# NVIDIA/cuopt

Measured on NVIDIA H100. Metric: pdlp_iterations_per_sec, higher is better.
Workload: dtype f64

## Files before the change

### cuopt_b200/csrc/pdlp_kernels.cuh

```cuda
#pragma once

#include "device_utils.cuh"
#include "spmv_bicsr.cuh"

#include <math_constants.h>

namespace cuopt_b200 {

constexpr int EW_THREADS  = 256;
static __device__ int g_l2_hints = 1;

struct pdhg_ctl_t {
  double step_size, primal_weight, tau, sigma;
  double pending_weight;
  double sum_weights;
  double interaction, norm_dx2, norm_dy2;
  double reduction_exponent, growth_exponent, primal_smoothing, dual_smoothing;
  int parity;
  int pending_avg;
  int active;
  int valid;
  int k_pdhg;
  int attempts;
  int accepted;
// ... 161 lines not shown
  const bool pending      = ctl->pending_avg != 0;
  const double w          = ctl->pending_weight;
  const int stride        = gridDim.x * blockDim.x;
  const l2_policy_t pol   = make_l2_policies(g_l2_hints);
  for (int j = blockIdx.x * blockDim.x + threadIdx.x; j < n; j += stride) {
    const double xj = x[j];
    if (pending) sum_x[j] = sum_x[j] + w * xj;
    const double gradient = ld_stream(c + j) - aty[j];
    double next           = xj - (tau * gradient);
    next                  = fmax(fmin(next, ld_stream(u + j)), ld_stream(l + j));
    xn[j]                 = next;
    st_l2(xbar + j, next - xj + next, pol.keep);
  }
}

template <bool INIT, int NPRE, bool BCAST = false>
__global__ void __launch_bounds__(BICSR_THREADS, bicsr_min_ctas(NPRE)) k_dual_step(pdhg_ctl_t* __restrict__ ctl,
                                                                             bicsr_view_t A,
                                                                             const double* __restrict__ xbar,
                                                                             double* __restrict__ ybuf0,
                                                                             double* __restrict__ ybuf1,
                                                                             const double* __restrict__ lc,
                                                                             const double* __restrict__ uc,
                                                                             double* __restrict__ sum_y,
                                                                             double* __restrict__ part_dy2,
                                                                             const unsigned long long* xbar_flags,
                                                                             int n_xbar_flags,
                                                                             const double* __restrict__ t,
                                                                             peer_ptrs_t y_peers = peer_ptrs_t{},
                                                                             peer_flags_t flags = peer_flags_t{},
                                                                             int world = 1,
// ... 32 lines not shown
    const double low = next + sigma * p.lc;
    const double up  = next + sigma * p.uc;
    next             = fmax(low, fmin(up, 0.0));
    st_l2(yn + i, next, pol.keep);
    if constexpr (BCAST) {
#pragma unroll
      for (int r = 0; r < DIST_MAX_PEERS; ++r)
        if (r < world) {
          const int d = __ldg(send + (size_t)r * send_stride + i);
          if (d >= 0) y_peers.p[r][d] = next;
        }
    }
    const double d   = next - p.y;
    dy2 += d * d;
  };
  spmv_bicsr_rows<payload_t, INIT, NPRE>(A, xbar, rows[threadIdx.x >> 5], pre_op, row_op, pol.keep);
  const double tot = block_reduce(dy2, red);
  if (threadIdx.x == 0) part_dy2[blockIdx.x] = tot;
  if constexpr (BCAST) peer_signal_grid_done(&ctl->ticket[2], flags, world, DIST_FLAG_Y + rank, epoch, DIST_FLAG_Y_B + rank);
}

template <bool INIT, int NPRE>
__global__ void __launch_bounds__(BICSR_THREADS, bicsr_min_ctas(NPRE)) k_transpose_step(pdhg_ctl_t* __restrict__ ctl,
                                                                                  bicsr_view_t AT,
                                                                                  const double* __restrict__ ybuf0,
                                                                                  const double* __restrict__ ybuf1,
                                                                                  const double* __restrict__ xbuf0,
                                                                                  const double* __restrict__ xbuf1,
                                                                                  double* __restrict__ aty0,
                                                                                  double* __restrict__ aty1,
                                                                                  double* __restrict__ parts,
                                                                                  const double* __restrict__ part_dy2,
                                                                                  int n_part_dy2,
                                                                                  const double* __restrict__ t)
{
  if (!ctl->active) return;
  __shared__ double rows[BICSR_WARPS][BICSR_SLOTS];
// ... 9 lines not shown
  struct payload_t {
    double dx, aty, init;
  };
  auto pre_op = [&](int j) {
    payload_t p;
    p.dx   = ld_l2(xn + j, pol.stream) - ld_l2(x + j, pol.stream);
    p.aty  = ld_l2(aty + j, pol.stream);
    p.init = INIT ? ld_l2(t + j, pol.stream) : 0.0;
    return p;
  };
  auto row_op = [&](int j, double s, const payload_t& p) {
    st_l2(atyn + j, s, pol.stream);
    acc[0] += p.dx * (s - p.aty);
    acc[1] += p.dx * p.dx;
  };
  spmv_bicsr_rows<payload_t, INIT, NPRE>(AT, yn, rows[threadIdx.x >> 5], pre_op, row_op, pol.keep);

  if (!publish_and_elect<2>(acc, parts, &ctl->ticket[0], red)) return;
  const double interaction = gather_partials(parts, gridDim.x, red);
  const double dx2         = gather_partials(parts + gridDim.x, gridDim.x, red);
  const double dy2         = gather_partials(part_dy2, n_part_dy2, red);
  if (threadIdx.x != 0) return;

  pdhg_step_rule(ctl, interaction, dx2, dy2);
}

template <bool INIT, int NPRE>
__global__ void __launch_bounds__(BICSR_THREADS, bicsr_min_ctas(NPRE)) k_transpose_step_slice(pdhg_ctl_t* __restrict__ ctl,
                                                                                        bicsr_view_t AT,
                                                                                        const double* __restrict__ yfull,
                                                                                        const double* __restrict__ xbuf0,
// ... 334 lines not shown
__global__ void k_step_rule_gather(pdhg_ctl_t* __restrict__ ctl, const double* __restrict__ scal, int n_src,
                                   const unsigned long long* wait_flags)
{
  if (!ctl->active) return;
  if (wait_flags) peer_wait(wait_flags, n_src, (unsigned long long)ctl->attempts + 1ull);
  if (threadIdx.x != 0) return;
  double interaction = 0.0, dx2 = 0.0, dy2 = 0.0;
  for (int g = 0; g < n_src; ++g) {
    interaction += __ldcg(scal + 4 * g + 0);
    dx2 += __ldcg(scal + 4 * g + 1);
    dy2 += __ldcg(scal + 4 * g + 2);
  }
  pdhg_step_rule(ctl, interaction, dx2, dy2);
}

__global__ void __launch_bounds__(BICSR_THREADS, BICSR_MIN_CTAS) k_block_pass(const pdhg_ctl_t* __restrict__ ctl,
                                                                              bicsr_view_t Ab,
                                                                              const double* __restrict__ x0,
                                                                              const double* __restrict__ x1,
                                                                              int pick_candidate,
                                                                              double* __restrict__ t,
                                                                              int first,
                                                                              const unsigned long long* wait_flags,
                                                                              int n_wait)
{
  if (!ctl->active) return;
  __shared__ double rows[BICSR_WARPS][BICSR_SLOTS];
  if (wait_flags) peer_wait(wait_flags, n_wait, (unsigned long long)ctl->attempts + 1ull);
  const double* x       = pick_candidate ? (ctl->parity ? x0 : x1) : x0;
  const l2_policy_t pol = make_l2_policies(g_l2_hints);
  struct payload_t {
    double init;
  };
  auto pre_op = [&](int r) {
    payload_t p;
    p.init = first ? 0.0 : ld_l2(t + r, pol.stream);
    return p;
  };
  auto row_op = [&](int r, double s, const payload_t&) { st_l2(t + r, s, pol.stream); };
  spmv_bicsr_rows<payload_t, true>(Ab, x, rows[threadIdx.x >> 5], pre_op, row_op, pol.keep);
}

__global__ void __launch_bounds__(EW_THREADS) k_flush_average(const pdhg_ctl_t* __restrict__ ctl,
                                                              int n,
                                                              const double* __restrict__ xbuf0,
                                                              const double* __restrict__ xbuf1,
                                                              double* __restrict__ sum_x,
                                                              int m,
                                                              const double* __restrict__ ybuf0,
                                                              const double* __restrict__ ybuf1,
                                                              double* __restrict__ sum_y)
{
  if (!ctl->pending_avg) return;
  const int cur    = ctl->parity;
  const double* x  = cur ? xbuf1 : xbuf0;
// ... 10 lines not shown
  ctl->valid  = 0;
  ctl->active = steps > 0 ? 1 : 0;
}

__global__ void __launch_bounds__(BICSR_THREADS, BICSR_MIN_CTAS) k_spmv(bicsr_view_t A,
                                                                        const double* __restrict__ x,
                                                                        double* __restrict__ out)
{
  __shared__ double rows[BICSR_WARPS][BICSR_SLOTS];
  struct payload_t {};
  auto pre_op = [&](int) { return payload_t{}; };
  auto row_op = [&](int i, double s, const payload_t&) { out[i] = s; };
  spmv_bicsr_rows<payload_t>(A, x, rows[threadIdx.x >> 5], pre_op, row_op, make_l2_policies(g_l2_hints).keep);
}

__global__ void __launch_bounds__(BICSR_THREADS, BICSR_MIN_CTAS) k_spmv_pair(bicsr_view_t M,
                                                                             const double* __restrict__ u,
                                                                             const double* __restrict__ v,
                                                                             double* __restrict__ out_u,
                                                                             double* __restrict__ out_v,
                                                                             int first)
{
  __shared__ double rows[2][BICSR_WARPS][BICSR_SLOTS];
  auto row_op = [&](int r, double su, double sv) {
    out_u[r] = first ? su : out_u[r] + su;
    out_v[r] = first ? sv : out_v[r] + sv;
  };
  const int w = threadIdx.x >> 5;
  spmv_bicsr_rows_pair(M, u, v, rows[0][w], rows[1][w], row_op, make_l2_policies(g_l2_hints).keep);
}

__device__ __forceinline__ double bound_value_product(double value, double lower, double upper)
{
  double bound = 0.0;
  if (value > 0.0) bound = lower;
  else if (value < 0.0) bound = upper;
  return isfinite(bound) ? value * bound : 0.0;
}

__device__ __forceinline__ void eval_column(int j, const double (&s)[2], double cj, double lo, double hi,
                                            const double (&xv)[2], int reduced_cost_rule, double* __restrict__ rc_cur,
                                            double* __restrict__ rc_avg, double (&acc)[8])
{
  double* rcs[2] = {rc_cur, rc_avg};
// ... 525 lines not shown
```

### cuopt_b200/csrc/pdlp_solver.cu

```cuda
#include "pdlp_solver.hpp"

#include "dist_comm.hpp"
#include "pdlp_kernels.cuh"
#include "presolve.cuh"
#include "trust_region.cuh"

#include <math_constants.h>
#include <nvtx3/nvToolsExt.h>

#include <algorithm>
#include <chrono>
#include <cmath>
#include <cstdio>
#include <cstdlib>
#include <atomic>
#include <map>
#include <mutex>
#include <thread>
#include <string>

namespace cuopt_b200 {

namespace {

struct bicsr_dev_t {
  int n_std = 0, n_blk = 0;
  dvec<int2> desc;
  dvec<unsigned short> row_slot;
  dvec<int> idx;
  dvec<double> val;
};

struct csr_dev_t {
  int rows = 0, cols = 0, nnz = 0;
  dvec<int> off, idx;
  dvec<double> val;
  bicsr_dev_t bi;
  const csr_dev_t* structure = nullptr;
  const int* off_ptr() const { return structure ? structure->off.data() : off.data(); }
  const int* idx_ptr() const { return structure ? structure->idx.data() : idx.data(); }
  const bicsr_dev_t& bi_structure() const { return structure ? structure->bi : bi; }
  int n_blk() const { return bi_structure().n_blk; }
  bicsr_view_t view() const
  {
    const bicsr_dev_t& s = bi_structure();
    return bicsr_view_t{s.desc.data(), s.row_slot.data(), s.idx.data(), bi.val.data(), s.n_std, s.n_blk,
                        off_ptr(),     idx_ptr(),         val.data()};
  }
  void alias_structure_copy_values(const csr_dev_t& o, cudaStream_t s)
  {
    rows = o.rows; cols = o.cols; nnz = o.nnz;
    structure = &o;
    val.copy_from(o.val, s);
  }
};

constexpr int SCHEDULE_SEGMENT = 1 << 16;
template <typename T, typename F>
std::vector<T> cut_in_segments(int rows, F cut_segment)
{
  const int n_seg = std::max(1, (rows + SCHEDULE_SEGMENT - 1) / SCHEDULE_SEGMENT);
  std::vector<std::vector<T>> part(n_seg);
// ... 55 lines not shown
  if (n_std > 0) {
    const int grid = std::max(1, std::min((n_std + 7) / 8, sms * 8));
    k_bicsr_fill<<<grid, 256, 0, s>>>(n_std, b.desc.data(), d.off.data(), d.idx.data(), d.val.data(), b.idx.data(),
                                      b.val.data(), b.row_slot.data());
    CUOPT_CUDA_TRY(cudaGetLastError());
  }
}
void fill_bicsr_values(csr_dev_t& d, cudaStream_t s, int sms)
{
  const bicsr_dev_t& st = d.bi_structure();
  d.bi.val.resize((size_t)std::max(st.n_std, 1) * BICSR_SLOTS);
  if (st.n_std > 0) {
    const int grid = std::max(1, std::min((st.n_std + 7) / 8, sms * 8));
    k_bicsr_fill_values<<<grid, 256, 0, s>>>(st.n_std, st.desc.data(), d.off_ptr(), d.val.data(), d.bi.val.data());
    CUOPT_CUDA_TRY(cudaGetLastError());
  }
}

template <typename VI, typename VD>
void upload_csr(csr_dev_t& d, int rows, int cols, const VI& off, const VI& idx, const VD& val, cudaStream_t s, int sms);

}

void csr_transpose_device(int rows, int cols, int nnz, const int* off, const int* idx, const double* val, int* toff,
                          int* tidx, double* tval, cudaStream_t stream);

void sort_keys_with_index(int count, const double* keys_in, double* keys_out, const int* vals_in, int* vals_out,
                          cudaStream_t stream);
void inclusive_sum_in_place(int count, double* values, cudaStream_t stream);
void exclusive_sum_int(int count, const int* in, int* out, cudaStream_t stream);
// ... 199 lines not shown
  void* xbar_peer[DIST_MAX_PEERS]  = {};
  void* scal_peer[DIST_MAX_PEERS]  = {};
  void* flag_peer[DIST_MAX_PEERS]  = {};
  bool peers_open = false;
  peer_ptrs_t p_xbar{}, p_scal{};
  peer_flags_t p_flags{};
  dvec<unsigned> d_ticket;
  dvec<pdhg_ctl_t> d_ctl;
  dvec<eval_t> d_eval;
  pdhg_ctl_t* h_ctl = nullptr;
  eval_t* h_eval    = nullptr;
  double* h_scalar  = nullptr;
  int occ_spmv = 1;
  int occ_spmv2 = 1;
  int npre_override = 0;
  dvec<double> eval_m, eval_n;
  dvec<double> part_max;
  dvec<double> part_infeas;
  bool tr_enabled = false;
  double tr_gap_reduction_last_trial = 1.0;
  int grid_tr = 1;
  dvec<double> tr_aty, tr_ax, tr_grad, tr_dir, tr_thr, tr_thr_sorted, tr_A, tr_B, tr_parts, tr_scal;
  dvec<int> tr_iota, tr_perm;
  struct tr_gap_t {
    const double *px, *py;
    double pd = 0, dd = 0, dist = 0, lower = 0, upper = 0, ngap = 0;
  };
  struct gather_blocks_t {
    int B = 1, width = 0;
    std::vector<csr_dev_t> blk;
    std::vector<csr_dev_t> unscaled;
    std::vector<int> grid;
    bool on() const { return B > 1; }
  };
  gather_blocks_t blkA, blkAT, blkATslice;
  dvec<double> t_m, t_n;
  size_t gather_block_bytes = 0;
  int n_part_dy2 = 1;
  int grid_k1 = 1, grid_k2 = 1, grid_k3 = 1, grid_n = 1, grid_m = 1, grid_misc = 1;
  long long staged_fills = 0;
  std::map<int, cudaGraphExec_t> graphs;
  bool use_graphs = true;
  cudaEvent_t ev_a = nullptr, ev_b = nullptr;

// ... 231 lines not shown
    }
    grid_k2   = spmv_grid(As);
    grid_k3   = spmv_grid(ATs);
    grid_n    = ew_grid(n, sms);
    grid_m    = ew_grid(m, sms);
    grid_k1   = grid_n;
    grid_misc = ew_grid(std::max(n, m), sms);
    part_dy2.resize((size_t)std::max({grid_k2, grid_m, sms * 16}));
    n_part_dy2 = grid_k2;
    {
      int l2 = 0;
      CUOPT_CUDA_TRY(cudaDeviceGetAttribute(&l2, cudaDevAttrL2CacheSize, dev));
      gather_block_bytes = (size_t)((double)l2 * GATHER_BLOCK_L2_FRACTION);
    }
    if (const char* e = std::getenv("CUOPT_B200_GATHER_BLOCK_BYTES")) gather_block_bytes = (size_t)std::atoll(e);
    part_k3.resize(2 * (size_t)std::max({grid_k3, grid_n, sms * 16}));
    part_rows.resize(6 * (size_t)grid_m);
    if (hp.restart_strategy == 2) {
      tr_enabled = true;
      {
        if (sharded())
          throw lp_error(error_type_t::ValidationError, "Methodical1 is not available in multi-GPU solves");
        const size_t N = (size_t)n + m;
        grid_tr        = ew_grid((int)std::min<size_t>(N, 1u << 30), sms);
        tr_aty.resize(n); tr_ax.resize(m); tr_grad.resize(N); tr_dir.resize(N); tr_thr.resize(N); tr_thr_sorted.resize(N);
        tr_A.resize(N); tr_B.resize(N); tr_iota.resize(N); tr_perm.resize(N);
        tr_parts.resize(5 * (size_t)grid_tr);
        tr_scal.resize(TR_SCALARS);
        tr_scal.zero(stream);
      }
// ... 462 lines not shown
    g = gather_blocks_t{};
    const size_t bytes = (size_t)M.cols * sizeof(double);
    int B              = 1;
    if (forced_width > 0) {
      if (M.nnz == 0 || M.rows == 0) return;
      g.width = forced_width;
      B       = 2;
    } else {
      if (gather_block_bytes == 0 || bytes <= gather_block_bytes + gather_block_bytes / 2 || M.nnz == 0) return;
      B       = (int)std::min<size_t>(16, (bytes + gather_block_bytes - 1) / gather_block_bytes);
      g.width = (((M.cols + B - 1) / B) + 31) & ~31;
      B       = (M.cols + g.width - 1) / g.width;
    }
    if (B <= 1) return;
    g.B = B;
    g.blk.resize(B);
    std::vector<int*> offs(B), idxs(B);
    std::vector<double*> vals(B);
    std::vector<int> nnz_b(B, 0);
    for (int b = 0; b < B; ++b) {
      g.blk[b].rows = M.rows;
      g.blk[b].cols = M.cols;
      g.blk[b].off.resize((size_t)M.rows + 1);
      offs[b] = g.blk[b].off.data();
    }
    csr_split_columns_offsets(M.rows, M.off_ptr(), M.idx_ptr(), g.width, B, offs.data(), nnz_b.data(), stream);
    for (int b = 0; b < B; ++b) {
      g.blk[b].nnz = nnz_b[b];
      g.blk[b].idx.resize((size_t)nnz_b[b]);
      g.blk[b].val.resize((size_t)nnz_b[b]);
      idxs[b] = g.blk[b].idx.data();
      vals[b] = g.blk[b].val.data();
    }
    csr_split_columns_fill(M.rows, M.off_ptr(), M.idx_ptr(), M.val.data(), g.width, B, offs.data(), idxs.data(), vals.data(),
                           stream);
    std::vector<int> hoff((size_t)M.rows + 1);
    g.grid.resize(B);
    for (int b = 0; b < B; ++b) {
      g.blk[b].off.download(hoff.data(), stream);
      sync();
      build_bicsr(g.blk[b], hoff, stream, sms);
      g.grid[b] = spmv_grid(g.blk[b]);
    }
    if (unscaled_src) {
      g.unscaled.resize(B);
      for (int b = 0; b < B; ++b) {
        csr_dev_t& U = g.unscaled[b];
        U.rows = M.rows; U.cols = M.cols; U.nnz = nnz_b[b];
        U.structure = &g.blk[b];
        U.val.resize((size_t)nnz_b[b]);
        vals[b] = U.val.data();
      }
      csr_split_columns_fill(M.rows, M.off_ptr(), M.idx_ptr(), unscaled_src->val.data(), g.width, B, offs.data(), idxs.data(),
                             vals.data(), stream);
      for (csr_dev_t& U : g.unscaled) {
        fill_bicsr_values(U, stream, sms);
        if (U.bi_structure().n_std == U.bi_structure().n_blk) {
          sync();
          U.val = dvec<double>{};
        }
      }
    }
    t.resize((size_t)M.rows);
    t.zero(stream);
  }
  void launch_block_passes(const gather_blocks_t& g, int count, const double* x0, const double* x1, int pick_candidate,
                           double* t, const unsigned long long* wait_flags, int n_wait)
  {
    for (int b = 0; b < count; ++b) {
      const csr_dev_t& M = g.blk[b];
      k_block_pass<<<g.grid[b], BICSR_THREADS, 0, stream>>>(d_ctl.data(), M.view(), x0, x1, pick_candidate, t, b == 0,
                                                            b == 0 ? wait_flags : nullptr, n_wait);
    }
  }
  void enqueue_k2(const unsigned long long* wait_flags, int n_wait, bool bcast = false,
                  const unsigned long long* wait_flags_b = nullptr)
  {
    const bool blocked  = blkA.on();
    const csr_dev_t& L  = blocked ? blkA.blk[blkA.B - 1] : hot_A();
    const int npre      = fused_npre(L);
    const int grid      = spmv_grid(L, npre);
    const double* t     = blocked ? t_m.data() : nullptr;
    const unsigned long long* wf = wait_flags_b ? wait_flags_b : (blocked ? nullptr : wait_flags);
    if (blocked) launch_block_passes(blkA, blkA.B - 1, xbar.data(), xbar.data(), 0, t_m.data(), wait_flags, n_wait);
#define CUOPT_K2(INIT, NPRE)                                                                                             \
  k_dual_step<INIT, NPRE><<<grid, BICSR_THREADS, 0, stream>>>(d_ctl.data(), L.view(), xbar.data(), ybuf[0].data(),       \
                                                              ybuf[1].data(), lcs.data(), ucs.data(), sum_y.data(),      \
                                                              part_dy2.data(), wf, n_wait, t)
#define CUOPT_K2B(INIT, NPRE)                                                                                            \
  k_dual_step<INIT, NPRE, true><<<grid, BICSR_THREADS, 0, stream>>>(d_ctl.data(), L.view(), xbar.data(), ybuf[0].data(), \
                                                                    ybuf[1].data(), lcs.data(), ucs.data(), sum_y.data(), \
                                                                    part_dy2.data(), wf, n_wait, t, p_yfull, p_flags,     \
                                                                    dist->world, dist->rank, sendY.data(), m)
    if (bcast) {
      if (blocked) { if (npre > 1) CUOPT_K2B(true, 2); else CUOPT_K2B(true, 1); }
      else { if (npre > 1) CUOPT_K2B(false, 2); else CUOPT_K2B(false, 1); }
    } else if (blocked) { if (npre > 1) CUOPT_K2(true, 2); else CUOPT_K2(true, 1); }
    else { if (npre > 1) CUOPT_K2(false, 2); else CUOPT_K2(false, 1); }
#undef CUOPT_K2B
#undef CUOPT_K2
  }
  int k2_grid() const
  {
    const csr_dev_t& L = blkA.on() ? blkA.blk[blkA.B - 1] : hot_A();
    return spmv_grid(L, fused_npre(L));
  }
  int k3_npre() const { return npre_override > 1 ? 2 : 1; }
  int k3_grid() const { return spmv_grid(blkAT.on() ? blkAT.blk[blkAT.B - 1] : ATs, k3_npre()); }
  void enqueue_k3()
  {
    const bool blocked = blkAT.on();
    const csr_dev_t& L = blocked ? blkAT.blk[blkAT.B - 1] : ATs;
    const int npre     = k3_npre();
    const int grid     = k3_grid();
    const double* t    = blocked ? t_n.data() : nullptr;
    if (blocked) launch_block_passes(blkAT, blkAT.B - 1, ybuf[0].data(), ybuf[1].data(), 1, t_n.data(), nullptr, 0);
#define CUOPT_K3(INIT, NPRE)                                                                                              \
  k_transpose_step<INIT, NPRE><<<grid, BICSR_THREADS, 0, stream>>>(d_ctl.data(), L.view(), ybuf[0].data(), ybuf[1].data(), \
                                                                   xbuf[0].data(), xbuf[1].data(), atybuf[0].data(),      \
                                                                   atybuf[1].data(), part_k3.data(), part_dy2.data(),     \
                                                                   n_part_dy2, t)
    if (blocked) { if (npre > 1) CUOPT_K3(true, 2); else CUOPT_K3(true, 1); }
    else { if (npre > 1) CUOPT_K3(false, 2); else CUOPT_K3(false, 1); }
#undef CUOPT_K3
  }
  int kernels_per_attempt() const
  {
    const int k2 = blkA.on() ? blkA.B : 1;
    if (!sharded()) return 1 + k2 + (blkAT.on() ? blkAT.B : 1);
    if (dist_gather) return 1 + k2 + (blkATslice.on() ? blkATslice.B : 1) + 1 + (dist_send_kernel ? 2 : 0);
    return 1 + k2 + (blkAT.on() ? blkAT.B : 1) + 2;
  }

  void launch_transpose_partial()
  {
    if (blkAT.on()) {
      launch_block_passes(blkAT, blkAT.B, ybuf[0].data(), ybuf[1].data(), 1, dist_buf.data(), nullptr, 0);
      return;
    }
    k_transpose_partial<<<grid_k3, BICSR_THREADS, 0, stream>>>(d_ctl.data(), ATs.view(), ybuf[0].data(), ybuf[1].data(),
                                                               dist_buf.data());
  }
  void launch_spmv(const csr_dev_t& M, const double* v, double* out)
  {
    k_spmv<<<spmv_grid(M), BICSR_THREADS, 0, stream>>>(M.view(), v, out);
  }
  int launch_spmv_pair(const csr_dev_t& M, const gather_blocks_t& g, const double* u, const double* v, double* out_u,
                       double* out_v)
  {
    const int count = g.unscaled.empty() ? 1 : (int)g.unscaled.size();
    for (int b = 0; b < count; ++b) {
      const csr_dev_t& Mb = g.unscaled.empty() ? M : g.unscaled[b];
      k_spmv_pair<<<spmv_grid(Mb), BICSR_THREADS, 0, stream>>>(Mb.view(), u, v, out_u, out_v, b == 0);
    }
    return count;
  }

  void enqueue_sliced_attempt()
  {
    const int j0 = slice_j0, G = dist->world, rk = dist->rank;
    double *x0 = xbuf[0].data() + j0, *x1 = xbuf[1].data() + j0, *a0 = atybuf[0].data() + j0, *a1 = atybuf[1].data() + j0;
    if (dist_gather) {
      const unsigned long long* fl = d_flags.data();
      tr_tick(0);
      if (dist_send_kernel) {
        k_primal_step<<<grid_slice, EW_THREADS, 0, stream>>>(d_ctl.data(), slice_n, x0, x1, a0, a1, cs.data() + j0,
                                                             ls.data() + j0, us.data() + j0, sum_x.data() + j0, xloc.data());
        CUOPT_CUDA_TRY(cudaEventRecord(ev_fork, stream));
// ... 710 lines not shown
  if (name == "sum_w") return k.sum_weights;
  if (name == "k_total") return s.total_pdlp_iterations;
  if (name == "k_pdhg") return k.attempts;
  if (name == "its_since_restart") return k.its_since_restart;
  if (name == "interaction") return k.interaction;
  if (name == "norm_dx2") return k.norm_dx2;
  if (name == "norm_dy2") return k.norm_dy2;
  if (name == "l2_norm_b") return s.l2_norm_b;
  if (name == "l2_norm_c") return s.l2_norm_c;
  if (name == "last_restart_kkt") return s.last_restart_kkt;
  if (name == "last_candidate_kkt") return s.last_candidate_kkt;
  if (name == "n_restarts") return s.sol.stats.n_restarts;
  if (name == "last_restart_was_average") return s.last_restart_was_average ? 1.0 : 0.0;
  if (name == "eval_blocks") return (double)std::max<size_t>(1, s.blkA.unscaled.size());
  if (name == "eval_blocks_t") return (double)std::max<size_t>(1, s.blkAT.unscaled.size());
  if (name == "valid") return k.valid;
  if (name == "sm_count") return s.sms;
  if (name == "occ_spmv") return s.occ_spmv;
  if (name == "occ_spmv2") return s.occ_spmv2;
  if (name == "grid_k1") return s.grid_k1;
  if (name == "grid_k2") return s.k2_grid();
  if (name == "grid_k3") return s.k3_grid();
  if (name == "grid_n") return s.grid_n;
  if (name == "grid_m") return s.grid_m;
  if (name == "k2_npre") return s.fused_npre(s.blkA.on() ? s.blkA.blk[s.blkA.B - 1] : s.hot_A());
  if (name == "n_std_a") return s.As.bi_structure().n_std;
  if (name == "n_blk_a") return s.As.bi_structure().n_blk;
  if (name == "n_std_at") return s.ATs.bi_structure().n_std;
  if (name == "n_blk_at") return s.ATs.bi_structure().n_blk;
  if (name == "staged_fills") return (double)s.staged_fills;
// ... 163 lines not shown
```

### cuopt_b200/csrc/spmv_bicsr.cuh

```cuda
#pragma once

#include "device_utils.cuh"

namespace cuopt_b200 {

constexpr int BICSR_CH              = 8;
constexpr int BICSR_SLOTS           = 32 * BICSR_CH;
constexpr int BICSR_MAX_ROWS        = 256;
constexpr int BICSR_THREADS         = 256;
constexpr int BICSR_WARPS           = BICSR_THREADS / 32;
constexpr int BICSR_PAD             = 0x7fffffff;
constexpr unsigned short BICSR_EMPTY = 0xffff;
constexpr int BICSR_MIN_CTAS        = 4;
__host__ __device__ constexpr int bicsr_min_ctas(int npre) { return npre > 1 ? 3 : BICSR_MIN_CTAS; }

__host__ __device__ constexpr int bicsr_slot(int q) { return (q % BICSR_CH) * 32 + q / BICSR_CH; }

struct bicsr_view_t {
  const int2* desc;
  const unsigned short* row_slot;
  const int* idx;
  const double* val;
  int n_std, n_blk;
  const int* off;
  const int* cidx;
  const double* cval;
};

__device__ __forceinline__ void bicsr_block_row_sums(const double (&a)[BICSR_CH], const double (&g)[BICSR_CH], unsigned ends,
                                                     int lane, double* rsw)
{
  constexpr unsigned FULL = 0xffffffffu;
  double s = 0.0, head = 0.0;
  const int kf = ends ? __ffs(ends) - 1 : -1;
#pragma unroll
  for (int k = 0; k < BICSR_CH; ++k) {
    s = __dadd_rn(s, __dmul_rn(a[k], g[k]));
    const bool e = (ends >> k) & 1u;
    if (e && k != kf) rsw[k * 32 + lane] = s;
    head = (k == kf) ? s : head;
    s    = e ? 0.0 : s;
  }
  double tail  = s;
  double carry = __shfl_up_sync(FULL, tail, 1);
  if (lane == 0) carry = 0.0;
  unsigned pending = __ballot_sync(FULL, kf < 0);
  while (pending) {
    if (kf < 0) tail = carry + s;
    carry = __shfl_up_sync(FULL, tail, 1);
    if (lane == 0) carry = 0.0;
    pending &= pending << 1;
  }
  if (kf >= 0) rsw[kf * 32 + lane] = carry + head;
}

template <typename P, bool INIT = false, int NPRE = 1, typename PreOp, typename RowOp>
__device__ __forceinline__ void spmv_bicsr_rows(const bicsr_view_t& A,
                                                const double* __restrict__ x,
                                                double* rsw,
                                                PreOp& pre_op,
                                                RowOp& row_op,
                                                unsigned long long gather_policy)
{
  const int lane          = threadIdx.x & 31;
  const int gwarp         = blockIdx.x * BICSR_WARPS + (threadIdx.x >> 5);
  const int nwarps        = gridDim.x * BICSR_WARPS;
  int c[BICSR_CH];
  if (gwarp < A.n_std) {
#pragma unroll
    for (int k = 0; k < BICSR_CH; ++k) c[k] = ld_stream(A.idx + (size_t)gwarp * BICSR_SLOTS + k * 32 + lane);
  }
  for (int b = gwarp; b < A.n_std; b += nwarps) {
    const int2 d  = __ldg(A.desc + b);
    const int r0 = d.x, r1 = d.y;
    P pl[NPRE];
    unsigned short slot[NPRE];
#pragma unroll
    for (int q = 0; q < NPRE; ++q) {
      slot[q] = BICSR_EMPTY;
      if (r0 + lane + 32 * q < r1) {
        pl[q]   = pre_op(r0 + lane + 32 * q);
        slot[q] = __ldg(A.row_slot + r0 + lane + 32 * q);
      }
    }
    const size_t base = (size_t)b * BICSR_SLOTS + lane;
    double a[BICSR_CH], g[BICSR_CH];
#pragma unroll
    for (int k = 0; k < BICSR_CH; ++k) a[k] = ld_stream(A.val + base + k * 32);
#pragma unroll
    for (int k = 0; k < BICSR_CH; ++k) {
      const int col = c[k] & 0x7fffffff;
      g[k]          = col != BICSR_PAD ? ld_l2(x + col, gather_policy) : 0.0;
    }
    unsigned ends = 0;
#pragma unroll
    for (int k = 0; k < BICSR_CH; ++k) ends |= (unsigned)(c[k] < 0) << k;
    if (b + nwarps < A.n_std) {
#pragma unroll
      for (int k = 0; k < BICSR_CH; ++k) c[k] = ld_stream(A.idx + (size_t)(b + nwarps) * BICSR_SLOTS + k * 32 + lane);
    }
    bicsr_block_row_sums(a, g, ends, lane, rsw);
    __syncwarp();
#pragma unroll
    for (int q = 0; q < NPRE; ++q) {
      if (r0 + lane + 32 * q < r1) {
        double sum = slot[q] != BICSR_EMPTY ? rsw[slot[q]] : 0.0;
        if constexpr (INIT) sum = pl[q].init + sum;
        row_op(r0 + lane + 32 * q, sum, pl[q]);
      }
    }
    for (int r = r0 + 32 * NPRE + lane; r < r1; r += 32) {
      const P p2              = pre_op(r);
      const unsigned short s2 = __ldg(A.row_slot + r);
      double sum              = s2 != BICSR_EMPTY ? rsw[s2] : 0.0;
      if constexpr (INIT) sum = p2.init + sum;
      row_op(r, sum, p2);
    }
    __syncwarp();
  }
  for (int b = A.n_std + gwarp; b < A.n_blk; b += nwarps) {
    const int row = __ldg(A.desc + b).x;
    const int lo = __ldg(A.off + row), hi = __ldg(A.off + row + 1);
    P pl;
    if (lane == 0) pl = pre_op(row);
    double acc = 0.0;
    for (int e = lo + lane; e < hi; e += 32) acc += ld_stream(A.cval + e) * ld_l2(x + ld_stream(A.cidx + e), gather_policy);
    acc = warp_sum(acc);
    if (lane == 0) {
      if constexpr (INIT) acc = pl.init + acc;
      row_op(row, acc, pl);
    }
  }
}

template <typename RowOp>
__device__ __forceinline__ void spmv_bicsr_rows_pair(const bicsr_view_t& A,
                                                     const double* __restrict__ u,
                                                     const double* __restrict__ v,
                                                     double* rsw_u,
                                                     double* rsw_v,
                                                     RowOp& row_op,
                                                     unsigned long long gather_policy)
{
  const int lane   = threadIdx.x & 31;
  const int gwarp  = blockIdx.x * BICSR_WARPS + (threadIdx.x >> 5);
  const int nwarps = gridDim.x * BICSR_WARPS;
  for (int b = gwarp; b < A.n_std; b += nwarps) {
    const int2 d      = __ldg(A.desc + b);
    const size_t base = (size_t)b * BICSR_SLOTS + lane;
    int c[BICSR_CH];
    double a[BICSR_CH], gu[BICSR_CH], gv[BICSR_CH];
#pragma unroll
    for (int k = 0; k < BICSR_CH; ++k) c[k] = ld_stream(A.idx + base + k * 32);
#pragma unroll
    for (int k = 0; k < BICSR_CH; ++k) a[k] = ld_stream(A.val + base + k * 32);
#pragma unroll
    for (int k = 0; k < BICSR_CH; ++k) {
      const int col = c[k] & 0x7fffffff;
      gu[k]         = col != BICSR_PAD ? ld_l2(u + col, gather_policy) : 0.0;
      gv[k]         = col != BICSR_PAD ? ld_l2(v + col, gather_policy) : 0.0;
    }
    unsigned ends = 0;
#pragma unroll
    for (int k = 0; k < BICSR_CH; ++k) ends |= (unsigned)(c[k] < 0) << k;
    bicsr_block_row_sums(a, gu, ends, lane, rsw_u);
    bicsr_block_row_sums(a, gv, ends, lane, rsw_v);
    __syncwarp();
    for (int r = d.x + lane; r < d.y; r += 32) {
      const unsigned short s = __ldg(A.row_slot + r);
      row_op(r, s != BICSR_EMPTY ? rsw_u[s] : 0.0, s != BICSR_EMPTY ? rsw_v[s] : 0.0);
    }
    __syncwarp();
  }
  for (int b = A.n_std + gwarp; b < A.n_blk; b += nwarps) {
    const int row = __ldg(A.desc + b).x;
    const int lo = __ldg(A.off + row), hi = __ldg(A.off + row + 1);
    double acc_u = 0.0, acc_v = 0.0;
    for (int e = lo + lane; e < hi; e += 32) {
      const double a = ld_stream(A.cval + e);
      const int col  = ld_stream(A.cidx + e);
      acc_u += a * ld_l2(u + col, gather_policy);
      acc_v += a * ld_l2(v + col, gather_policy);
    }
    acc_u = warp_sum(acc_u);
    acc_v = warp_sum(acc_v);
// ... 43 lines not shown
{
  const int lane = threadIdx.x & 31, wpb = blockDim.x >> 5;
  for (int b = blockIdx.x * wpb + (threadIdx.x >> 5); b < n_std; b += gridDim.x * wpb) {
    const int2 d      = desc[b];
    const int lo      = off[d.x];
    const int cnt     = off[d.y] - lo;
    const size_t base = (size_t)b * BICSR_SLOTS;
#pragma unroll
    for (int k = 0; k < BICSR_CH; ++k) {
      const int q                = BICSR_CH * lane + k;
      bval[base + k * 32 + lane] = q < cnt ? val[lo + q] : 0.0;
    }
  }
}

}
```

Baseline: 366.1.

## Compact block-CSR column indices to 24-bit and replace row slots with bitmasks

```diff
diff --git a/cuopt_b200/csrc/pdlp_kernels.cuh b/cuopt_b200/csrc/pdlp_kernels.cuh
--- a/cuopt_b200/csrc/pdlp_kernels.cuh
+++ b/cuopt_b200/csrc/pdlp_kernels.cuh
@@ -199,7 +199,7 @@
   }
 }
 
-template <bool INIT, int NPRE, bool BCAST = false>
+template <bool INIT, int NPRE, bool BCAST = false, int FMT = 0>
 __global__ void __launch_bounds__(BICSR_THREADS, bicsr_min_ctas(NPRE)) k_dual_step(pdhg_ctl_t* __restrict__ ctl,
                                                                              bicsr_view_t A,
                                                                              const double* __restrict__ xbar,
@@ -262,13 +262,13 @@
     const double d   = next - p.y;
     dy2 += d * d;
   };
-  spmv_bicsr_rows<payload_t, INIT, NPRE>(A, xbar, rows[threadIdx.x >> 5], pre_op, row_op, pol.keep);
+  spmv_bicsr_rows<payload_t, INIT, NPRE, FMT>(A, xbar, rows[threadIdx.x >> 5], pre_op, row_op, pol.keep);
   const double tot = block_reduce(dy2, red);
   if (threadIdx.x == 0) part_dy2[blockIdx.x] = tot;
   if constexpr (BCAST) peer_signal_grid_done(&ctl->ticket[2], flags, world, DIST_FLAG_Y + rank, epoch, DIST_FLAG_Y_B + rank);
 }
 
-template <bool INIT, int NPRE>
+template <bool INIT, int NPRE, int FMT = 0>
 __global__ void __launch_bounds__(BICSR_THREADS, bicsr_min_ctas(NPRE)) k_transpose_step(pdhg_ctl_t* __restrict__ ctl,
                                                                                   bicsr_view_t AT,
                                                                                   const double* __restrict__ ybuf0,
@@ -308,7 +308,7 @@
     acc[0] += p.dx * (s - p.aty);
     acc[1] += p.dx * p.dx;
   };
-  spmv_bicsr_rows<payload_t, INIT, NPRE>(AT, yn, rows[threadIdx.x >> 5], pre_op, row_op, pol.keep);
+  spmv_bicsr_rows<payload_t, INIT, NPRE, FMT>(AT, yn, rows[threadIdx.x >> 5], pre_op, row_op, pol.keep);
 
   if (!publish_and_elect<2>(acc, parts, &ctl->ticket[0], red)) return;
   const double interaction = gather_partials(parts, gridDim.x, red);
@@ -673,6 +673,7 @@
   pdhg_step_rule(ctl, interaction, dx2, dy2);
 }
 
+template <int FMT = 0>
 __global__ void __launch_bounds__(BICSR_THREADS, BICSR_MIN_CTAS) k_block_pass(const pdhg_ctl_t* __restrict__ ctl,
                                                                               bicsr_view_t Ab,
                                                                               const double* __restrict__ x0,
@@ -697,7 +698,7 @@
     return p;
   };
   auto row_op = [&](int r, double s, const payload_t&) { st_l2(t + r, s, pol.stream); };
-  spmv_bicsr_rows<payload_t, true>(Ab, x, rows[threadIdx.x >> 5], pre_op, row_op, pol.keep);
+  spmv_bicsr_rows<payload_t, true, 1, FMT>(Ab, x, rows[threadIdx.x >> 5], pre_op, row_op, pol.keep);
 }
 
 __global__ void __launch_bounds__(EW_THREADS) k_flush_average(const pdhg_ctl_t* __restrict__ ctl,
@@ -738,6 +739,7 @@
   spmv_bicsr_rows<payload_t>(A, x, rows[threadIdx.x >> 5], pre_op, row_op, make_l2_policies(g_l2_hints).keep);
 }
 
+template <int FMT = 0>
 __global__ void __launch_bounds__(BICSR_THREADS, BICSR_MIN_CTAS) k_spmv_pair(bicsr_view_t M,
                                                                              const double* __restrict__ u,
                                                                              const double* __restrict__ v,
@@ -751,7 +753,7 @@
     out_v[r] = first ? sv : out_v[r] + sv;
   };
   const int w = threadIdx.x >> 5;
-  spmv_bicsr_rows_pair(M, u, v, rows[0][w], rows[1][w], row_op, make_l2_policies(g_l2_hints).keep);
+  spmv_bicsr_rows_pair<FMT>(M, u, v, rows[0][w], rows[1][w], row_op, make_l2_policies(g_l2_hints).keep);
 }
 
 __device__ __forceinline__ double bound_value_product(double value, double lower, double upper)
diff --git a/cuopt_b200/csrc/pdlp_solver.cu b/cuopt_b200/csrc/pdlp_solver.cu
--- a/cuopt_b200/csrc/pdlp_solver.cu
+++ b/cuopt_b200/csrc/pdlp_solver.cu
@@ -25,10 +25,14 @@
 
 struct bicsr_dev_t {
   int n_std = 0, n_blk = 0;
+  int fmt = 0, col0 = 0;
   dvec<int2> desc;
   dvec<unsigned short> row_slot;
   dvec<int> idx;
   dvec<double> val;
+  dvec<unsigned short> lo16;
+  dvec<unsigned long long> hi8;
+  dvec<unsigned> mask;
 };
 
 struct csr_dev_t {
@@ -44,8 +48,8 @@
   bicsr_view_t view() const
   {
     const bicsr_dev_t& s = bi_structure();
-    return bicsr_view_t{s.desc.data(), s.row_slot.data(), s.idx.data(), bi.val.data(), s.n_std, s.n_blk,
-                        off_ptr(),     idx_ptr(),         val.data()};
+    return bicsr_view_t{s.desc.data(), s.row_slot.data(), s.idx.data(), bi.val.data(), s.n_std,  s.n_blk, off_ptr(),
+                        idx_ptr(),     val.data(),        s.lo16.data(), s.hi8.data(), s.mask.data(), s.col0};
   }
   void alias_structure_copy_values(const csr_dev_t& o, cudaStream_t s)
   {
@@ -131,6 +135,38 @@
     const int grid = std::max(1, std::min((st.n_std + 7) / 8, sms * 8));
     k_bicsr_fill_values<<<grid, 256, 0, s>>>(st.n_std, st.desc.data(), d.off_ptr(), d.val.data(), d.bi.val.data());
     CUOPT_CUDA_TRY(cudaGetLastError());
+  }
+}
+
+void compact_bicsr(csr_dev_t& d, int fmt, int col0, cudaStream_t s, int sms)
+{
+  bicsr_dev_t& b = d.bi;
+  b.fmt  = fmt;
+  b.col0 = col0;
+  if (fmt == 0 || b.n_std == 0) return;
+  const size_t ns = (size_t)b.n_std;
+  if (fmt & BICSR_FMT_IDX3) {
+    b.lo16.resize(ns * BICSR_SLOTS);
+    b.hi8.resize(ns * 32);
+  }
+  if (fmt & BICSR_FMT_MASK) b.mask.resize(ns * 8);
+  const int grid = std::max(1, std::min((b.n_std + BICSR_WARPS - 1) / BICSR_WARPS, sms * 8));
+  k_bicsr_fill_structure<<<grid, BICSR_THREADS, 0, s>>>(b.n_std, b.desc.data(), d.off.data(), d.idx.data(), col0,
+                                                        b.lo16.data(), b.hi8.data(), b.mask.data());
+  CUOPT_CUDA_TRY(cudaGetLastError());
+  CUOPT_CUDA_TRY(cudaStreamSynchronize(s));
+  if (fmt & BICSR_FMT_IDX3) b.idx = dvec<int>{};
+  if (fmt & BICSR_FMT_MASK) b.row_slot = dvec<unsigned short>{};
+}
+
+template <typename F>
+void with_fmt(int fmt, F&& f)
+{
+  switch (fmt) {
+    case BICSR_FMT_IDX3: f(std::integral_constant<int, BICSR_FMT_IDX3>{}); break;
+    case BICSR_FMT_MASK: f(std::integral_constant<int, BICSR_FMT_MASK>{}); break;
+    case BICSR_FMT_IDX3 | BICSR_FMT_MASK: f(std::integral_constant<int, BICSR_FMT_IDX3 | BICSR_FMT_MASK>{}); break;
+    default: f(std::integral_constant<int, 0>{});
   }
 }
 
@@ -360,6 +396,7 @@
   int occ_spmv = 1;
   int occ_spmv2 = 1;
   int npre_override = 0;
+  int compact_blocks = BICSR_FMT_IDX3 | BICSR_FMT_MASK;
   dvec<double> eval_m, eval_n;
   dvec<double> part_max;
   dvec<double> part_infeas;
@@ -374,6 +411,7 @@
   };
   struct gather_blocks_t {
     int B = 1, width = 0;
+    int fmt = 0;
     std::vector<csr_dev_t> blk;
     std::vector<csr_dev_t> unscaled;
     std::vector<int> grid;
@@ -635,6 +673,7 @@
       gather_block_bytes = (size_t)((double)l2 * GATHER_BLOCK_L2_FRACTION);
     }
     if (const char* e = std::getenv("CUOPT_B200_GATHER_BLOCK_BYTES")) gather_block_bytes = (size_t)std::atoll(e);
+    if (const char* e = std::getenv("CUOPT_B200_COMPACT_BLOCKS")) compact_blocks = std::atoi(e) & (BICSR_FMT_IDX3 | BICSR_FMT_MASK);
     part_k3.resize(2 * (size_t)std::max({grid_k3, grid_n, sms * 16}));
     part_rows.resize(6 * (size_t)grid_m);
     if (hp.restart_strategy == 2) {
@@ -1127,6 +1166,10 @@
     }
     if (B <= 1) return;
     g.B = B;
+    if (forced_width == 0 && !sharded()) {
+      g.fmt = compact_blocks;
+      if (g.width > BICSR_IDX3_MAX_WIDTH) g.fmt &= ~BICSR_FMT_IDX3;
+    }
     g.blk.resize(B);
     std::vector<int*> offs(B), idxs(B);
     std::vector<double*> vals(B);
@@ -1153,6 +1196,7 @@
       g.blk[b].off.download(hoff.data(), stream);
       sync();
       build_bicsr(g.blk[b], hoff, stream, sms);
+      compact_bicsr(g.blk[b], g.fmt, b * g.width, stream, sms);
       g.grid[b] = spmv_grid(g.blk[b]);
     }
     if (unscaled_src) {
@@ -1182,8 +1226,10 @@
   {
     for (int b = 0; b < count; ++b) {
       const csr_dev_t& M = g.blk[b];
-      k_block_pass<<<g.grid[b], BICSR_THREADS, 0, stream>>>(d_ctl.data(), M.view(), x0, x1, pick_candidate, t, b == 0,
-                                                            b == 0 ? wait_flags : nullptr, n_wait);
+      with_fmt(g.fmt, [&](auto F) {
+        k_block_pass<decltype(F)::value><<<g.grid[b], BICSR_THREADS, 0, stream>>>(
+          d_ctl.data(), M.view(), x0, x1, pick_candidate, t, b == 0, b == 0 ? wait_flags : nullptr, n_wait);
+      });
     }
   }
   void enqueue_k2(const unsigned long long* wait_flags, int n_wait, bool bcast = false,
@@ -1196,10 +1242,10 @@
     const double* t     = blocked ? t_m.data() : nullptr;
     const unsigned long long* wf = wait_flags_b ? wait_flags_b : (blocked ? nullptr : wait_flags);
     if (blocked) launch_block_passes(blkA, blkA.B - 1, xbar.data(), xbar.data(), 0, t_m.data(), wait_flags, n_wait);
-#define CUOPT_K2(INIT, NPRE)                                                                                             \
-  k_dual_step<INIT, NPRE><<<grid, BICSR_THREADS, 0, stream>>>(d_ctl.data(), L.view(), xbar.data(), ybuf[0].data(),       \
-                                                              ybuf[1].data(), lcs.data(), ucs.data(), sum_y.data(),      \
-                                                              part_dy2.data(), wf, n_wait, t)
+#define CUOPT_K2(INIT, NPRE, FMT)                                                                                        \
+  k_dual_step<INIT, NPRE, false, FMT><<<grid, BICSR_THREADS, 0, stream>>>(                                               \
+    d_ctl.data(), L.view(), xbar.data(), ybuf[0].data(), ybuf[1].data(), lcs.data(), ucs.data(), sum_y.data(),          \
+    part_dy2.data(), wf, n_wait, t)
 #define CUOPT_K2B(INIT, NPRE)                                                                                            \
   k_dual_step<INIT, NPRE, true><<<grid, BICSR_THREADS, 0, stream>>>(d_ctl.data(), L.view(), xbar.data(), ybuf[0].data(), \
                                                                     ybuf[1].data(), lcs.data(), ucs.data(), sum_y.data(), \
@@ -1208,8 +1254,11 @@
     if (bcast) {
       if (blocked) { if (npre > 1) CUOPT_K2B(true, 2); else CUOPT_K2B(true, 1); }
       else { if (npre > 1) CUOPT_K2B(false, 2); else CUOPT_K2B(false, 1); }
-    } else if (blocked) { if (npre > 1) CUOPT_K2(true, 2); else CUOPT_K2(true, 1); }
-    else { if (npre > 1) CUOPT_K2(false, 2); else CUOPT_K2(false, 1); }
+    } else if (blocked) {
+      with_fmt(blkA.fmt, [&](auto F) {
+        if (npre > 1) CUOPT_K2(true, 2, decltype(F)::value); else CUOPT_K2(true, 1, decltype(F)::value);
+      });
+    } else { if (npre > 1) CUOPT_K2(false, 2, 0); else CUOPT_K2(false, 1, 0); }
 #undef CUOPT_K2B
 #undef CUOPT_K2
   }
@@ -1228,13 +1277,15 @@
     const int grid     = k3_grid();
     const double* t    = blocked ? t_n.data() : nullptr;
     if (blocked) launch_block_passes(blkAT, blkAT.B - 1, ybuf[0].data(), ybuf[1].data(), 1, t_n.data(), nullptr, 0);
-#define CUOPT_K3(INIT, NPRE)                                                                                              \
-  k_transpose_step<INIT, NPRE><<<grid, BICSR_THREADS, 0, stream>>>(d_ctl.data(), L.view(), ybuf[0].data(), ybuf[1].data(), \
-                                                                   xbuf[0].data(), xbuf[1].data(), atybuf[0].data(),      \
-                                                                   atybuf[1].data(), part_k3.data(), part_dy2.data(),     \
-                                                                   n_part_dy2, t)
-    if (blocked) { if (npre > 1) CUOPT_K3(true, 2); else CUOPT_K3(true, 1); }
-    else { if (npre > 1) CUOPT_K3(false, 2); else CUOPT_K3(false, 1); }
+#define CUOPT_K3(INIT, NPRE, FMT)                                                                                         \
+  k_transpose_step<INIT, NPRE, FMT><<<grid, BICSR_THREADS, 0, stream>>>(                                                  \
+    d_ctl.data(), L.view(), ybuf[0].data(), ybuf[1].data(), xbuf[0].data(), xbuf[1].data(), atybuf[0].data(),            \
+    atybuf[1].data(), part_k3.data(), part_dy2.data(), n_part_dy2, t)
+    if (blocked) {
+      with_fmt(blkAT.fmt, [&](auto F) {
+        if (npre > 1) CUOPT_K3(true, 2, decltype(F)::value); else CUOPT_K3(true, 1, decltype(F)::value);
+      });
+    } else { if (npre > 1) CUOPT_K3(false, 2, 0); else CUOPT_K3(false, 1, 0); }
 #undef CUOPT_K3
   }
   int kernels_per_attempt() const
@@ -1264,7 +1315,9 @@
     const int count = g.unscaled.empty() ? 1 : (int)g.unscaled.size();
     for (int b = 0; b < count; ++b) {
       const csr_dev_t& Mb = g.unscaled.empty() ? M : g.unscaled[b];
-      k_spmv_pair<<<spmv_grid(Mb), BICSR_THREADS, 0, stream>>>(Mb.view(), u, v, out_u, out_v, b == 0);
+      with_fmt(g.fmt, [&](auto F) {
+        k_spmv_pair<decltype(F)::value><<<spmv_grid(Mb), BICSR_THREADS, 0, stream>>>(Mb.view(), u, v, out_u, out_v, b == 0);
+      });
     }
     return count;
   }
@@ -2005,6 +2058,8 @@
   if (name == "last_restart_was_average") return s.last_restart_was_average ? 1.0 : 0.0;
   if (name == "eval_blocks") return (double)std::max<size_t>(1, s.blkA.unscaled.size());
   if (name == "eval_blocks_t") return (double)std::max<size_t>(1, s.blkAT.unscaled.size());
+  if (name == "blocks_form_a") return s.blkA.fmt;
+  if (name == "blocks_form_at") return s.blkAT.fmt;
   if (name == "valid") return k.valid;
   if (name == "sm_count") return s.sms;
   if (name == "occ_spmv") return s.occ_spmv;
diff --git a/cuopt_b200/csrc/spmv_bicsr.cuh b/cuopt_b200/csrc/spmv_bicsr.cuh
--- a/cuopt_b200/csrc/spmv_bicsr.cuh
+++ b/cuopt_b200/csrc/spmv_bicsr.cuh
@@ -16,6 +16,12 @@
 
 __host__ __device__ constexpr int bicsr_slot(int q) { return (q % BICSR_CH) * 32 + q / BICSR_CH; }
 
+constexpr int BICSR_FMT_IDX3     = 1;
+constexpr int BICSR_FMT_MASK     = 2;
+constexpr int BICSR_IDX3_MAX_WIDTH = 1 << 21;
+constexpr unsigned BICSR_HI_PAD  = 0x40u;
+constexpr unsigned BICSR_HI_END  = 0x80u;
+
 struct bicsr_view_t {
   const int2* desc;
   const unsigned short* row_slot;
@@ -25,19 +31,102 @@
   const int* off;
   const int* cidx;
   const double* cval;
+  const unsigned short* lo16;
+  const unsigned long long* hi8;
+  const unsigned* mask;
+  int col0;
 };
 
+template <int FMT>
+struct bicsr_cols_t {
+  int c[BICSR_CH];
+};
+template <>
+struct bicsr_cols_t<BICSR_FMT_IDX3> {
+  uint4 lo;
+  unsigned long long hi;
+};
+template <>
+struct bicsr_cols_t<BICSR_FMT_IDX3 | BICSR_FMT_MASK> : bicsr_cols_t<BICSR_FMT_IDX3> {};
+template <>
+struct bicsr_cols_t<BICSR_FMT_MASK> : bicsr_cols_t<0> {};
+
+template <int FMT>
+__device__ __forceinline__ void bicsr_load_cols(const bicsr_view_t& A, int b, int lane, bicsr_cols_t<FMT>& w)
+{
+  if constexpr ((FMT & BICSR_FMT_IDX3) != 0) {
+    w.lo = __ldcs(reinterpret_cast<const uint4*>(A.lo16 + (size_t)b * BICSR_SLOTS) + lane);
+    w.hi = __ldcs(A.hi8 + (size_t)b * 32 + lane);
+  } else {
+#pragma unroll
+    for (int k = 0; k < BICSR_CH; ++k) w.c[k] = ld_stream(A.idx + (size_t)b * BICSR_SLOTS + k * 32 + lane);
+  }
+}
+template <int FMT>
+__device__ __forceinline__ int bicsr_col(const bicsr_cols_t<FMT>& w, int k)
+{
+  if constexpr ((FMT & BICSR_FMT_IDX3) != 0) {
+    const unsigned lw = k < 2 ? w.lo.x : k < 4 ? w.lo.y : k < 6 ? w.lo.z : w.lo.w;
+    const unsigned hb = (unsigned)(w.hi >> (8 * k)) & 0xffu;
+    return (hb & BICSR_HI_PAD) ? -1 : (int)(((hb & 0x1fu) << 16) | ((lw >> (16 * (k & 1))) & 0xffffu));
+  } else {
+    const int col = w.c[k] & 0x7fffffff;
+    return col != BICSR_PAD ? col : -1;
+  }
+}
+template <int FMT>
+__device__ __forceinline__ unsigned bicsr_ends(const bicsr_cols_t<FMT>& w)
+{
+  unsigned ends = 0;
+#pragma unroll
+  for (int k = 0; k < BICSR_CH; ++k) {
+    if constexpr ((FMT & BICSR_FMT_IDX3) != 0) ends |= (unsigned)((w.hi >> (8 * k + 7)) & 1u) << k;
+    else ends |= (unsigned)(w.c[k] < 0) << k;
+  }
+  return ends;
+}
+template <int FMT>
+__device__ __forceinline__ const double* bicsr_gather_base(const bicsr_view_t& A, const double* x)
+{
+  if constexpr ((FMT & BICSR_FMT_IDX3) != 0) return x + A.col0;
+  else return x;
+}
+
+struct bicsr_mask_cursor_t {
+  unsigned mw;
+  int base;
+  __device__ __forceinline__ int next(int q, int lane)
+  {
+    const unsigned m = __shfl_sync(0xffffffffu, mw, q);
+    const int ord    = ((m >> lane) & 1u) ? base + __popc(m & ((1u << lane) - 1u)) : -1;
+    base += __popc(m);
+    return ord;
+  }
+};
+
+__device__ __forceinline__ int bicsr_ends_before(unsigned ends, int lane)
+{
+  const unsigned cnt = __popc(ends), lt = (1u << lane) - 1u;
+  int before         = 0;
+#pragma unroll
+  for (int j = 0; j < 4; ++j) before += __popc(__ballot_sync(0xffffffffu, (cnt >> j) & 1u) & lt) << j;
+  return before;
+}
+
+template <bool MASK = false>
 __device__ __forceinline__ void bicsr_block_row_sums(const double (&a)[BICSR_CH], const double (&g)[BICSR_CH], unsigned ends,
-                                                     int lane, double* rsw)
+                                                     int lane, double* rsw, int before = 0)
 {
   constexpr unsigned FULL = 0xffffffffu;
   double s = 0.0, head = 0.0;
   const int kf = ends ? __ffs(ends) - 1 : -1;
+  int ord      = before;
 #pragma unroll
   for (int k = 0; k < BICSR_CH; ++k) {
     s = __dadd_rn(s, __dmul_rn(a[k], g[k]));
     const bool e = (ends >> k) & 1u;
-    if (e && k != kf) rsw[k * 32 + lane] = s;
+    if (e && k != kf) rsw[MASK ? ord : k * 32 + lane] = s;
+    if constexpr (MASK) ord += e;
     head = (k == kf) ? s : head;
     s    = e ? 0.0 : s;
   }
@@ -51,10 +140,10 @@
     if (lane == 0) carry = 0.0;
     pending &= pending << 1;
   }
-  if (kf >= 0) rsw[kf * 32 + lane] = carry + head;
-}
-
-template <typename P, bool INIT = false, int NPRE = 1, typename PreOp, typename RowOp>
+  if (kf >= 0) rsw[MASK ? before : kf * 32 + lane] = carry + head;
+}
+
+template <typename P, bool INIT = false, int NPRE = 1, int FMT = 0, typename PreOp, typename RowOp>
 __device__ __forceinline__ void spmv_bicsr_rows(const bicsr_view_t& A,
                                                 const double* __restrict__ x,
                                                 double* rsw,
@@ -62,25 +151,25 @@
                                                 RowOp& row_op,
                                                 unsigned long long gather_policy)
 {
+  constexpr bool MASK     = (FMT & BICSR_FMT_MASK) != 0;
   const int lane          = threadIdx.x & 31;
   const int gwarp         = blockIdx.x * BICSR_WARPS + (threadIdx.x >> 5);
   const int nwarps        = gridDim.x * BICSR_WARPS;
-  int c[BICSR_CH];
-  if (gwarp < A.n_std) {
-#pragma unroll
-    for (int k = 0; k < BICSR_CH; ++k) c[k] = ld_stream(A.idx + (size_t)gwarp * BICSR_SLOTS + k * 32 + lane);
-  }
+  const double* xg        = bicsr_gather_base<FMT>(A, x);
+  bicsr_cols_t<FMT> c;
+  if (gwarp < A.n_std) bicsr_load_cols<FMT>(A, gwarp, lane, c);
   for (int b = gwarp; b < A.n_std; b += nwarps) {
     const int2 d  = __ldg(A.desc + b);
     const int r0 = d.x, r1 = d.y;
     P pl[NPRE];
     unsigned short slot[NPRE];
+    bicsr_mask_cursor_t mc{0u, 0};
 #pragma unroll
     for (int q = 0; q < NPRE; ++q) {
       slot[q] = BICSR_EMPTY;
       if (r0 + lane + 32 * q < r1) {
-        pl[q]   = pre_op(r0 + lane + 32 * q);
-        slot[q] = __ldg(A.row_slot + r0 + lane + 32 * q);
+        pl[q] = pre_op(r0 + lane + 32 * q);
+        if constexpr (!MASK) slot[q] = __ldg(A.row_slot + r0 + lane + 32 * q);
       }
     }
     const size_t base = (size_t)b * BICSR_SLOTS + lane;
@@ -89,32 +178,38 @@
     for (int k = 0; k < BICSR_CH; ++k) a[k] = ld_stream(A.val + base + k * 32);
 #pragma unroll
     for (int k = 0; k < BICSR_CH; ++k) {
-      const int col = c[k] & 0x7fffffff;
-      g[k]          = col != BICSR_PAD ? ld_l2(x + col, gather_policy) : 0.0;
-    }
-    unsigned ends = 0;
-#pragma unroll
-    for (int k = 0; k < BICSR_CH; ++k) ends |= (unsigned)(c[k] < 0) << k;
-    if (b + nwarps < A.n_std) {
-#pragma unroll
-      for (int k = 0; k < BICSR_CH; ++k) c[k] = ld_stream(A.idx + (size_t)(b + nwarps) * BICSR_SLOTS + k * 32 + lane);
-    }
-    bicsr_block_row_sums(a, g, ends, lane, rsw);
+      const int col = bicsr_col<FMT>(c, k);
+      g[k]          = col >= 0 ? ld_l2(xg + col, gather_policy) : 0.0;
+    }
+    if constexpr (MASK) mc.mw = lane < 8 ? __ldg(A.mask + (size_t)b * 8 + lane) : 0u;
+    const unsigned ends = bicsr_ends<FMT>(c);
+    if (b + nwarps < A.n_std) bicsr_load_cols<FMT>(A, b + nwarps, lane, c);
+    bicsr_block_row_sums<MASK>(a, g, ends, lane, rsw, MASK ? bicsr_ends_before(ends, lane) : 0);
     __syncwarp();
 #pragma unroll
     for (int q = 0; q < NPRE; ++q) {
+      int src = slot[q] != BICSR_EMPTY ? (int)slot[q] : -1;
+      if constexpr (MASK) src = mc.next(q, lane);
       if (r0 + lane + 32 * q < r1) {
-        double sum = slot[q] != BICSR_EMPTY ? rsw[slot[q]] : 0.0;
+        double sum = src >= 0 ? rsw[src] : 0.0;
         if constexpr (INIT) sum = pl[q].init + sum;
         row_op(r0 + lane + 32 * q, sum, pl[q]);
       }
     }
-    for (int r = r0 + 32 * NPRE + lane; r < r1; r += 32) {
-      const P p2              = pre_op(r);
-      const unsigned short s2 = __ldg(A.row_slot + r);
-      double sum              = s2 != BICSR_EMPTY ? rsw[s2] : 0.0;
-      if constexpr (INIT) sum = p2.init + sum;
-      row_op(r, sum, p2);
+    for (int q = NPRE; 32 * q < r1 - r0; ++q) {
+      const int r = r0 + 32 * q + lane;
+      int src     = -1;
+      if constexpr (MASK) src = mc.next(q, lane);
+      if (r < r1) {
+        const P p2 = pre_op(r);
+        if constexpr (!MASK) {
+          const unsigned short s2 = __ldg(A.row_slot + r);
+          src                     = s2 != BICSR_EMPTY ? (int)s2 : -1;
+        }
+        double sum = src >= 0 ? rsw[src] : 0.0;
+        if constexpr (INIT) sum = p2.init + sum;
+        row_op(r, sum, p2);
+      }
     }
     __syncwarp();
   }
@@ -133,7 +228,7 @@
   }
 }
 
-template <typename RowOp>
+template <int FMT = 0, typename RowOp>
 __device__ __forceinline__ void spmv_bicsr_rows_pair(const bicsr_view_t& A,
                                                      const double* __restrict__ u,
                                                      const double* __restrict__ v,
@@ -142,33 +237,44 @@
                                                      RowOp& row_op,
                                                      unsigned long long gather_policy)
 {
+  constexpr bool MASK = (FMT & BICSR_FMT_MASK) != 0;
   const int lane   = threadIdx.x & 31;
   const int gwarp  = blockIdx.x * BICSR_WARPS + (threadIdx.x >> 5);
   const int nwarps = gridDim.x * BICSR_WARPS;
+  const double* ug = bicsr_gather_base<FMT>(A, u);
+  const double* vg = bicsr_gather_base<FMT>(A, v);
   for (int b = gwarp; b < A.n_std; b += nwarps) {
     const int2 d      = __ldg(A.desc + b);
     const size_t base = (size_t)b * BICSR_SLOTS + lane;
-    int c[BICSR_CH];
+    bicsr_cols_t<FMT> c;
     double a[BICSR_CH], gu[BICSR_CH], gv[BICSR_CH];
-#pragma unroll
-    for (int k = 0; k < BICSR_CH; ++k) c[k] = ld_stream(A.idx + base + k * 32);
+    bicsr_load_cols<FMT>(A, b, lane, c);
+    bicsr_mask_cursor_t mc{0u, 0};
 #pragma unroll
     for (int k = 0; k < BICSR_CH; ++k) a[k] = ld_stream(A.val + base + k * 32);
 #pragma unroll
     for (int k = 0; k < BICSR_CH; ++k) {
-      const int col = c[k] & 0x7fffffff;
-      gu[k]         = col != BICSR_PAD ? ld_l2(u + col, gather_policy) : 0.0;
-      gv[k]         = col != BICSR_PAD ? ld_l2(v + col, gather_policy) : 0.0;
-    }
-    unsigned ends = 0;
-#pragma unroll
-    for (int k = 0; k < BICSR_CH; ++k) ends |= (unsigned)(c[k] < 0) << k;
-    bicsr_block_row_sums(a, gu, ends, lane, rsw_u);
-    bicsr_block_row_sums(a, gv, ends, lane, rsw_v);
-    __syncwarp();
-    for (int r = d.x + lane; r < d.y; r += 32) {
-      const unsigned short s = __ldg(A.row_slot + r);
-      row_op(r, s != BICSR_EMPTY ? rsw_u[s] : 0.0, s != BICSR_EMPTY ? rsw_v[s] : 0.0);
+      const int col = bicsr_col<FMT>(c, k);
+      gu[k]         = col >= 0 ? ld_l2(ug + col, gather_policy) : 0.0;
+      gv[k]         = col >= 0 ? ld_l2(vg + col, gather_policy) : 0.0;
+    }
+    const unsigned ends = bicsr_ends<FMT>(c);
+    const int before    = MASK ? bicsr_ends_before(ends, lane) : 0;
+    bicsr_block_row_sums<MASK>(a, gu, ends, lane, rsw_u, before);
+    bicsr_block_row_sums<MASK>(a, gv, ends, lane, rsw_v, before);
+    if constexpr (MASK) mc.mw = lane < 8 ? __ldg(A.mask + (size_t)b * 8 + lane) : 0u;
+    __syncwarp();
+    for (int q = 0; 32 * q < d.y - d.x; ++q) {
+      const int r = d.x + 32 * q + lane;
+      int s       = -1;
+      if constexpr (MASK) s = mc.next(q, lane);
+      if (r < d.y) {
+        if constexpr (!MASK) {
+          const unsigned short s2 = __ldg(A.row_slot + r);
+          s                       = s2 != BICSR_EMPTY ? (int)s2 : -1;
+        }
+        row_op(r, s >= 0 ? rsw_u[s] : 0.0, s >= 0 ? rsw_v[s] : 0.0);
+      }
     }
     __syncwarp();
   }
@@ -242,4 +348,53 @@
   }
 }
 
-}
+__global__ void __launch_bounds__(BICSR_THREADS) k_bicsr_fill_structure(int n_std,
+                                                                      const int2* __restrict__ desc,
+                                                                      const int* __restrict__ off,
+                                                                      const int* __restrict__ idx,
+                                                                      int col0,
+                                                                      unsigned short* __restrict__ lo16,
+                                                                      unsigned long long* __restrict__ hi8,
+                                                                      unsigned* __restrict__ mask)
+{
+  __shared__ unsigned char is_end[BICSR_WARPS][BICSR_SLOTS];
+  const int lane = threadIdx.x & 31, w = threadIdx.x >> 5;
+  unsigned char* e = is_end[w];
+  for (int b = blockIdx.x * BICSR_WARPS + w; b < n_std; b += gridDim.x * BICSR_WARPS) {
+    const int2 d      = desc[b];
+    const int lo      = off[d.x];
+    const int cnt     = off[d.y] - lo;
+    const size_t base = (size_t)b * BICSR_SLOTS;
+#pragma unroll
+    for (int k = 0; k < BICSR_CH; ++k) e[BICSR_CH * lane + k] = 0;
+    __syncwarp();
+    for (int q = 0; q < BICSR_MAX_ROWS / 32; ++q) {
+      const int r  = d.x + 32 * q + lane;
+      const int p0 = r < d.y ? off[r] : 0, p1 = r < d.y ? off[r + 1] : 0;
+      if (p1 > p0) e[p1 - 1 - lo] = 1;
+      const unsigned word = __ballot_sync(0xffffffffu, p1 > p0);
+      if (mask && lane == 0) mask[(size_t)b * 8 + q] = word;
+    }
+    __syncwarp();
+    if (lo16) {
+      unsigned lw[4] = {0u, 0u, 0u, 0u};
+      unsigned long long hw = 0ull;
+#pragma unroll
+      for (int k = 0; k < BICSR_CH; ++k) {
+        const int q = BICSR_CH * lane + k;
+        unsigned hb = BICSR_HI_PAD;
+        if (q < cnt) {
+          const unsigned c = (unsigned)(idx[lo + q] - col0);
+          lw[k / 2] |= (c & 0xffffu) << (16 * (k & 1));
+          hb = (c >> 16) | (e[q] ? BICSR_HI_END : 0u);
+        }
+        hw |= (unsigned long long)hb << (8 * k);
+      }
+      reinterpret_cast<uint4*>(lo16 + base)[lane] = make_uint4(lw[0], lw[1], lw[2], lw[3]);
+      hi8[(size_t)b * 32 + lane]                  = hw;
+    }
+    __syncwarp();
+  }
+}
+
+}
```

Measured after the change: 399.1, median of 6. +9.0%, better.
